# JialeTao/MRFA

Measured on AMD Instinct MI355X. Metric: frames/sec (256x256 source+driving pair) fwd+bwd, higher is better.
Workload: dtype f32; 1 GPU; vox1.yaml MTIA (TokenPose_B) prior + DenseMotion + RaftFlow refinement, 256x256, bs=8/GPU, fwd+bwd+clip+Adam, train-mode BN, surrogate L1 loss; global_batch=8, parallelism=dp1, prior=mtia, background_predictor=False, sync_bn=False, launch=hipGraph, optimizer=FlatAdam (K20), mfma=bf16x6

## Files before the change

mrfa_amd/build.py:

```python
import glob
import os
import subprocess
import sys

HERE = os.path.dirname(os.path.abspath(__file__))
ROOT = os.path.dirname(HERE)
CSRC = os.path.join(HERE, "csrc")
LIBDIR = os.path.join(HERE, "_lib")
LIB = os.path.join(LIBDIR, "libmrfa_hip.so")
SOURCES = ["error.cpp", "conv_plan.hip", "conv_mfma.hip", "conv_split.hip", "conv_halo.hip", "conv_small.hip", "conv_lean.hip", "wgrad_mfma.hip", "wgrad_split.hip", "wgrad_halo.hip", "wgrad_small.hip", "wgrad_lean.hip", "conv_fewout.hip", "conv_fewout3.hip", "layout.hip", "pack_multi.hip", "norm.hip", "sample.hip", "elementwise.hip", "optim.hip", "tokenpose.hip", "attention_mfma.hip", "losses.hip", "prior.hip", "pose.hip", "metrics.hip", "frames.hip"]
FLAGS = ["--offload-arch=gfx950", "-O3", "-std=c++17", "-fPIC", "-I" + os.path.join(ROOT, "include"), "-I" + CSRC,
         "-Wno-unused-result"]


def _stale(out, deps):
    if not os.path.exists(out):
        return True
    t = os.path.getmtime(out)
    return any(os.path.getmtime(d) > t for d in deps)


def build(force: bool = False, verbose: bool = True) -> str:
    os.makedirs(LIBDIR, exist_ok=True)
    hipcc = os.environ.get("HIPCC", "/opt/rocm/bin/hipcc")
    headers = [os.path.join(ROOT, "include", h) for h in ("mrfa_hip.h", "mrfa_hip_ext.h")] + sorted(glob.glob(os.path.join(CSRC, "*.h")))
# ... 28 lines not shown
```

mrfa_amd/csrc/common.h:

```cpp
#pragma once
#include <hip/hip_runtime.h>
#include <stdio.h>
#include <string.h>
#include "mrfa_hip.h"

typedef float f32x16 __attribute__((ext_vector_type(16)));
typedef float f32x4 __attribute__((ext_vector_type(4)));

void mrfa_set_error(const char* fmt, ...);

struct MrfaTuning {
    int conv_small_env;
    int conv_small;
    int conv_halo, conv_halo_min_tiles, conv_halo_pr, conv_halo_phase, conv_halo_bn256, conv_halo_bn192, conv_halo_bn64_fill;
    int conv_lean, conv_lean_min_wgs, conv_lean_geo, gemm_lean;
    int wgrad_halo, wgrad_halo_min_wgs, wgrad_halo_target_wgs, wgrad_halo_phase, wgrad_lean;
    int conv_fewout3, attention_mfma, split_target_256;
};
extern MrfaTuning g_tune;

struct HaloGeo { int PR, BN; bool phase; };

enum class ConvFamily { lean, gemm_lean, small, halo, halo_dgrad, rows_split, rows_f32, refused };
struct ConvPlan {
    ConvFamily family;
    char error[256];
    long long M;
    int KT;
    int lean_geo, gemm_cfg, small_tm, small_tn;
    HaloGeo halo;
    int BM, BN, splitk;
    bool w8;
    bool fused;
    bool fin_in_launch;
    bool reads_w;
    int last_config;
    bool groups_ok, bst_ok, stride2_ok, mask_ok, phase_dgrad_ok;
};
ConvPlan plan_conv(const mrfa_conv_params& p);

enum class WgradFamily { lean, small, halo, tiled, refused };
struct WgradPlan {
    WgradFamily family;
    char error[192];
    long long M;
    bool lean, small;
    bool groups_ok, stride2_ok;
};
WgradPlan plan_wgrad(const mrfa_wgrad_params& p);

int mrfa_conv_split_launch(hipStream_t st, const mrfa_conv_params& p, int KT, long long M, int splitk, int BN);
bool mrfa_conv_halo_eligible(const mrfa_conv_params& p, HaloGeo* geo);
int mrfa_conv_halo_launch(hipStream_t st, const mrfa_conv_params& p, const HaloGeo& geo);
int mrfa_wgrad_split_launch(hipStream_t st, const mrfa_wgrad_params& p, dim3 grid, long long M, long long kps, int tiles_n, int nsplit, int inner,
                            int total_splits, int taps, long long partial_stride, int BM, int BN);

bool mrfa_wgrad_halo_eligible(const mrfa_wgrad_params& p);
int mrfa_wgrad_halo_launch(hipStream_t st, const mrfa_wgrad_params& p);

bool mrfa_fewout3_wgrad(hipStream_t st, const float* x, int ldx, int N, int H, int W, int Cin, const float* dy, int lddy, int Cout, int R, int pad,
                        float* dw, float* dbias, int* rc);

int mrfa_conv_lean_pick(const mrfa_conv_params& p);
int mrfa_conv_lean_launch(hipStream_t st, const mrfa_conv_params& p, int geo);
int mrfa_gemm_lean_pick(const mrfa_conv_params& p, long long M);
int mrfa_gemm_lean_launch(hipStream_t st, const mrfa_conv_params& p, long long M, int cfg);

bool mrfa_conv_small_eligible(const mrfa_conv_params& p, long long M);
int mrfa_conv_small_launch(hipStream_t st, const mrfa_conv_params& p, long long M, int tm, int tn);

bool mrfa_attention_mfma_ok(int d, int n, const void* qkv, int ld, const void* out, int ldo, const void* dout, int lddo, const void* dqkv, int lddq);
int mrfa_attention_fwd_mfma(hipStream_t st, const float* qkv, int ld, int B, int n, int heads, int d, float scale, float* out, int ldo, float* lse);
int mrfa_attention_bwd_mfma(hipStream_t st, const float* qkv, int ld, const float* out, int ldo, const float* dout, int lddo, const float* lse,
                            float* delta, int B, int n, int heads, int d, float scale, float* dqkv, int lddq);

bool mrfa_wgrad_lean_eligible(const mrfa_wgrad_params& p);
int mrfa_wgrad_lean_multi(hipStream_t st, const mrfa_wgrad_params* ps, int n, unsigned char* taken);

bool mrfa_wgrad_small_eligible(const mrfa_wgrad_params& p, long long M);
int mrfa_wgrad_small_launch(hipStream_t st, const mrfa_wgrad_params& p, long long M);

#define MRFA_CHECK_ARG(cond, ...)                      \
    do {                                               \
        if (!(cond)) {                                 \
// ... 123 lines not shown
```

mrfa_amd/csrc/conv_mfma.hip:

```cpp
#include "common.h"
#include <stdlib.h>

namespace {

constexpr int BK = 32;
constexpr int LDK = BK + 4;

template <int BM, int BN, int WAVES_M, int WAVES_N, bool FLAT>
__global__ __launch_bounds__(WAVES_M * WAVES_N * 64) void conv_mfma_kernel(const mrfa_conv_params p, const int KT, const int kt_per_split,
                                                       const long long M, const int tiles_n, const int total_tiles) {
    constexpr int TM = BM / WAVES_M / 32;
    constexpr int TN = BN / WAVES_N / 32;
    constexpr int NT = WAVES_M * WAVES_N * 64;
    constexpr int RSTEP = NT / 8;
    constexpr int RA = BM / RSTEP;
    constexpr int RB = BN / RSTEP;
    static_assert(WAVES_M * WAVES_N == 4 || WAVES_M * WAVES_N == 8, "4 or 8 waves");
    static_assert(RA >= 1 && RB >= 1, "tile too small for the workgroup");
    static_assert(TM >= 1 && TN >= 1, "tile");

    __shared__ __attribute__((aligned(16))) float smem[2 * (BM + BN) * LDK];

    const int tid = threadIdx.x;
    const int lane = tid & 63;
// ... 375 lines not shown
    }
    if (p.bst_x) {
        MRFA_CHECK_ARG(p.stats && p.bst_scale && p.bst_shift && p.bst_mean && p.bst_invstd && !p.fin_scale,
                       "conv2d: bst_x needs stats, bst_scale / _shift / _mean / _invstd and no fin_*");
        MRFA_CHECK_ARG(c.bst_ok, "conv2d: bst_* is only implemented by the small-problem kernels: ask mrfa_conv2d_bwdstats_supported() first");
    }
    MRFA_CHECK_ARG(p.y, "conv2d: null pointer");
    if (c.family == ConvFamily::refused) { mrfa_set_error("%s", c.error); return 1; }
    int rc;
    switch (c.family) {
        case ConvFamily::lean: g_last_tile = c.last_config; rc = mrfa_conv_lean_launch(st, p, c.lean_geo); break;
        case ConvFamily::gemm_lean: g_last_tile = c.last_config; rc = mrfa_gemm_lean_launch(st, p, c.M, c.gemm_cfg); break;
        case ConvFamily::small: g_last_tile = c.last_config; rc = mrfa_conv_small_launch(st, p, c.M, c.small_tm, c.small_tn); break;
        case ConvFamily::halo:
        case ConvFamily::halo_dgrad: g_last_tile = c.last_config; rc = mrfa_conv_halo_launch(st, p, c.halo); break;
        default: rc = launch_rows(st, p, c); break;
    }
    if (rc || !p.fin_scale || c.fin_in_launch) return rc;
    return mrfa_bn_finalize_groups(stream, p.stats, p.fin_count, p.fin_gamma, p.fin_beta, p.fin_rmean, p.fin_rvar, p.fin_momentum, p.fin_eps,
                                   p.Cout, p.groups > 1 ? p.groups : 1, p.fin_scale, p.fin_shift, p.fin_mean, p.fin_invstd);
}
```

mrfa_amd/csrc/conv_plan.hip:

```cpp
#include "common.h"
#include <stdarg.h>
#include <stdlib.h>

namespace {
int env_int(const char* name, int dflt) { const char* e = getenv(name); return e ? atoi(e) : dflt; }
int env_on(const char* name) { const char* e = getenv(name); return !(e && e[0] == '0'); }
}

MrfaTuning g_tune = {
     env_on("MRFA_CONV_SMALL"),  1,
     env_on("MRFA_CONV_HALO"),  128,  0,  1,  1,
     1,  1,
     env_on("MRFA_CONV_LEAN"),  128,  -1,
     env_int("MRFA_GEMM_LEAN", 1),
     env_on("MRFA_WGRAD_HALO"),  192,  256,  1,
     env_on("MRFA_WGRAD_LEAN"),
     1,  env_on("MRFA_ATTENTION_MFMA"),  env_int("MRFA_SPLIT_TARGET_256", 1),
};

enum TuneKind { T_ON, T_INT, T_NONNEG, T_NONNEG_ON, T_LEVEL, T_POS };
static const struct { const char* key; int* field; TuneKind kind; } TUNING_KEYS[] = {
    {"conv_small", &g_tune.conv_small, T_ON},
    {"conv_halo", &g_tune.conv_halo, T_ON},
    {"conv_halo_min_tiles", &g_tune.conv_halo_min_tiles, T_INT},
    {"conv_halo_pr", &g_tune.conv_halo_pr, T_INT},
    {"conv_halo_phase", &g_tune.conv_halo_phase, T_ON},
    {"conv_halo_bn256", &g_tune.conv_halo_bn256, T_ON},
    {"conv_halo_bn192", &g_tune.conv_halo_bn192, T_ON},
    {"conv_halo_bn64_fill", &g_tune.conv_halo_bn64_fill, T_ON},
    {"conv_lean", &g_tune.conv_lean, T_ON},
    {"conv_lean_min_wgs", &g_tune.conv_lean_min_wgs, T_NONNEG},
    {"conv_lean_geo", &g_tune.conv_lean_geo, T_INT},
    {"gemm_lean", &g_tune.gemm_lean, T_LEVEL},
    {"wgrad_halo", &g_tune.wgrad_halo, T_ON},
    {"wgrad_halo_min_wgs", &g_tune.wgrad_halo_min_wgs, T_NONNEG},
    {"wgrad_halo_target_wgs", &g_tune.wgrad_halo_target_wgs, T_POS},
    {"wgrad_halo_phase", &g_tune.wgrad_halo_phase, T_NONNEG_ON},
    {"wgrad_lean", &g_tune.wgrad_lean, T_ON},
    {"conv_fewout3", &g_tune.conv_fewout3, T_ON},
    {"attention_mfma", &g_tune.attention_mfma, T_ON},
};

extern "C" int mrfa_set_tuning(const char* key, int value) {
    if (!key) return -1;
    for (const auto& k : TUNING_KEYS) {
        if (strcmp(key, k.key)) continue;
        const int prev = *k.field;
        switch (k.kind) {
            case T_ON: *k.field = value != 0; break;
            case T_INT: *k.field = value; break;
            case T_NONNEG: if (value >= 0) *k.field = value; break;
            case T_NONNEG_ON: if (value >= 0) *k.field = value != 0; break;
            case T_LEVEL: if (value >= 0) *k.field = value > 2 ? 2 : value; break;
            case T_POS: if (value > 0) *k.field = value; break;
        }
// ... 84 lines not shown
ConvPlan plan_conv(const mrfa_conv_params& p) {
    ConvPlan c = {};
    const int mode = mrfa_get_mfma_mode();
    const bool flat = p.kflat > 0;
    c.M = (long long)p.N * p.Hout * p.Wout;
    c.KT = ((flat ? p.kflat : p.R * p.S * p.Cin) + BK - 1) / BK;
    c.splitk = 1;
    c.reads_w = true;
    c.fin_in_launch = p.fin_scale != nullptr;

    c.lean_geo = flat ? -1 : mrfa_conv_lean_pick(p);
    c.gemm_cfg = (flat || c.lean_geo >= 0) ? -1 : mrfa_gemm_lean_pick(p, c.M);
    const bool lean = c.lean_geo >= 0, gemm = c.gemm_cfg >= 0;
    const bool small = !lean && !gemm && g_tune.conv_small_env && g_tune.conv_small && mrfa_conv_small_eligible(p, c.M);
    const bool halo = !flat && mrfa_conv_halo_eligible(p, &c.halo);

    const long long rows = group_rows(p, c.M);
    c.groups_ok = p.groups <= 1 || !(p.stats || p.fin_scale || p.bst_x || p.in_scale) ||
                  (p.nbatch <= 1 && p.splitk <= 1 && rows > 0 &&
                   (lean || gemm || (!p.in_scale && ((rows % 128) == 0 || small || (p.stride <= 1 && halo)))));
    c.bst_ok = p.stats && !p.fin_scale && p.stride >= 0 && !flat && (lean || gemm || small);
    c.stride2_ok = p.stride == 2 && p.Hout == (p.Hin + 2 * p.pad - p.R) / 2 + 1 && p.Wout == (p.Win + 2 * p.pad - p.S) / 2 + 1 &&
                   (flat ? (!p.ups && p.nbatch <= 1 && p.splitk <= 1 && p.ktab) : small);
    c.mask_ok = halo;
    c.phase_dgrad_ok = p.ups == 2 && halo;

    if (!(p.x && p.w)) return refuse(c, "conv2d: null pointer");
    if (!(p.N > 0 && p.Cin > 0 && p.Cout > 0 && p.Hout > 0 && p.Wout > 0)) return refuse(c, "conv2d: bad sizes");
    if (!(p.R >= 1 && p.S >= 1 && p.R <= 15 && p.S <= 15)) return refuse(c, "conv2d: kernel size %dx%d unsupported", p.R, p.S);
    if (!((p.w_ld % 4) == 0 && aligned16(p.w))) return refuse(c, "conv2d: packed weight must be 16-B aligned, w_ld %% 4 == 0");
// ... 26 lines not shown
        c.small_tn = tn;
        c.last_config = (16 << 16) | (16 << 4) | 8;
        return c;
    }
    if (p.stride < 0 || p.stride > 2 || (p.stride == 2 && !(flat && !p.ups && p.nbatch <= 1)))
        return refuse(c, "conv2d: stride = %d is only implemented by the one-wave-per-tile kernel and by flat-K launches: ask mrfa_conv2d_stride_supported() first", p.stride);
    if (p.mask && !halo) return refuse(c, "conv2d: `mask` is only honoured by the patch-tiled kernel: ask mrfa_conv2d_mask_supported() first");
    if (p.ups == 2 && !halo)
        return refuse(c, "conv2d: ups = 2 (phase data gradient of a fused-upsample layer) is only implemented for the shapes mrfa_conv2d_phase_dgrad_supported() reports");
    if (halo) {
        c.family = p.ups == 2 ? ConvFamily::halo_dgrad : ConvFamily::halo;
        c.reads_w = false;
        c.last_config = (128 << 16) | ((p.Cout <= 64 ? 64 : 128) << 4) | 4 | (1 << 28);
        return c;
    }
    plan_rows(c, p, mode);
    return c;
}

WgradPlan plan_wgrad(const mrfa_wgrad_params& p) {
    WgradPlan c = {};
    const bool flat = p.kflat > 0;
    c.M = (long long)p.N * p.Hout * p.Wout;
    c.lean = mrfa_wgrad_lean_eligible(p);
    c.small = g_tune.conv_small_env && g_tune.conv_small && mrfa_wgrad_small_eligible(p, c.M);
    c.groups_ok = p.groups <= 1 || !p.in_scale || c.lean;
    c.stride2_ok = p.stride == 2 && p.Hout == (p.Hin + 2 * p.pad - p.R) / 2 + 1 && p.Wout == (p.Win + 2 * p.pad - p.S) / 2 + 1 && c.small;
    if (!(p.x && p.dy && p.dw)) return refuse(c, "wgrad: null pointer");
    if (!flat && !((p.ldx % 4) == 0 && aligned16(p.x))) return refuse(c, "wgrad: x must be a 16-B aligned view with ld %% 4 == 0");
    if (flat && !p.ktab) return refuse(c, "wgrad: flat mode needs ktab");
    if (!(c.M < (1ll << 31) - 64)) return refuse(c, "wgrad: too many pixels");
    if (p.in_scale && c.lean) { c.family = WgradFamily::lean; return c; }
    if (!c.groups_ok) return refuse(c, "wgrad: groups = %d with a prologue is only implemented where mrfa_conv2d_wgrad_groups_supported() says so", p.groups);
    if (c.small) { c.family = WgradFamily::small; return c; }
    if (p.stride > 1) return refuse(c, "wgrad: stride = %d is only implemented by the small-problem kernel: ask mrfa_conv2d_wgrad_stride_supported() first", p.stride);
    c.family = !flat && mrfa_wgrad_halo_eligible(p) ? WgradFamily::halo : WgradFamily::tiled;
    return c;
}

extern "C" int mrfa_conv2d_split_k(const mrfa_conv_params* p) {
    if (!p) return 1;
    if (p->splitk > 1) return p->splitk;
    const ConvPlan c = plan_conv(*p);
// ... 19 lines not shown
```

mrfa_amd/csrc/pack_multi.hip:

```cpp
#include <type_traits>
#include "mfma_bf16.h"

namespace {

constexpr int TCI = 32;
constexpr int MAXD = MRFA_PACK_MAX_DESCS;
constexpr int LDS_FLOATS = 12832;

struct PackArgs {
    int n;
    int tile_prefix[MAXD + 1];
    mrfa_pack_desc d[MAXD];
};

__host__ __device__ inline int tco_for(int T) { return T <= 9 ? 32 : (T <= 25 ? 16 : 8); }
__host__ __device__ inline int rup(int a, int b) { return (a + b - 1) / b * b; }

__device__ __forceinline__ long long dst_index(int mode, int co, int ci, int t, int Cout, int Cin, int T) {
    switch (mode) {
        case 0: return ((long long)t * rup(Cout, 128) + co) * rup(Cin, 32) + ci;
        case 1: return (long long)co * rup(T * Cin, 32) + t * Cin + ci;
        case 2: return ((long long)(T - 1 - t) * rup(Cin, 128) + ci) * rup(Cout, 32) + co;
        case 3: return (long long)ci * rup(T * Cout, 32) + (T - 1 - t) * Cout + co;
        case 5: return ((long long)co * T + t) * Cin + ci;
        default: return ((long long)ci * T + (T - 1 - t)) * Cout + co;
    }
}

__device__ __forceinline__ long long chunk_major(int tt, int r, int f, int rowsP, int colsP) {
    return (long long)tt * rowsP * colsP + (long long)(f >> 4) * (rowsP * 16) + r * 16 + (f & 15);
}

__device__ __forceinline__ int find_desc(const int* prefix, int n, int b) {
    int lo = 0, hi = n - 1;
    while (lo < hi) {
        const int mid = (lo + hi + 1) >> 1;
        if (prefix[mid] <= b) lo = mid; else hi = mid - 1;
    }
    return lo;
}

__global__ __launch_bounds__(256) void pack_multi_kernel(const PackArgs a) {
    __shared__ float lds[LDS_FLOATS];
    const int di = find_desc(a.tile_prefix, a.n, blockIdx.x);
    const mrfa_pack_desc& d = a.d[di];
    const int T = d.R * d.S, Cout = d.Cout, Cin = d.Cin;
    const int TCO = tco_for(T);
    const int tiles_ci = (Cin + TCI - 1) / TCI;
    const int tile = blockIdx.x - a.tile_prefix[di];
    const int co0 = (tile / tiles_ci) * TCO, ci0 = (tile % tiles_ci) * TCI;
    const int nco = min(TCO, Cout - co0), nci = min(TCI, Cin - ci0);
    const int row = TCI * T + 1;
    const int seg = nci * T;
    for (int i = threadIdx.x; i < nco * seg; i += 256) {
        const int co_l = i / seg, r = i - co_l * seg;
        lds[co_l * row + r] = d.src[((size_t)(co0 + co_l) * Cin + ci0) * T + r];
    }
    __syncthreads();
    for (int k = 0; k < d.ndst; ++k) {
        const int mode = d.mode[k];
        float* __restrict__ dst = d.dst[k];
        if (mode == 12 || mode == 13) {
            constexpr unsigned RM[4] = {0x1u, 0x6u, 0x3u, 0x4u};
            const bool tr = mode == 13;
            unsigned short* __restrict__ d16 = reinterpret_cast<unsigned short*>(dst);
            const int rowsP = tr ? rup(Cin, 128) : rup(Cout, 128), colsP = tr ? rup(Cout, 32) : rup(Cin, 32);
            const long long piece = 16ll * rowsP * colsP;
            const int nfast = tr ? nco : nci, nslow = tr ? nci : nco;
            const int f0 = (threadIdx.x & 15) * 2;
            for (int q = threadIdx.x >> 4; q < nslow * 16; q += 16) {
                const int sl = q >> 4, pt = q & 15;
                if (f0 >= nfast) continue;
                const int ph = pt >> 2, a_ = (pt >> 1) & 1, b_ = pt & 1;
                const unsigned rm = RM[(ph >> 1) * 2 + a_], sm = RM[(ph & 1) * 2 + b_];
                float v[2] = {0.f, 0.f};
#pragma unroll
                for (int e = 0; e < 2; ++e) {
                    if (f0 + e < nfast) {
                        const int co_l = tr ? f0 + e : sl, ci_l = tr ? sl : f0 + e;
                        const float* wl = lds + co_l * row + ci_l * T;
#pragma unroll
                        for (int r = 0; r < 3; ++r)
#pragma unroll
                            for (int s_ = 0; s_ < 3; ++s_)
                                if (((rm >> r) & 1u) && ((sm >> s_) & 1u)) v[e] += wl[r * 3 + s_];
                    }
                }
                const long long idx = tr ? chunk_major(pt, ci0 + sl, co0 + f0, rowsP, colsP) : chunk_major(pt, co0 + sl, ci0 + f0, rowsP, colsP);
                float x0 = v[0], x1 = v[1];
#pragma unroll
                for (int pc = 0; pc < 3; ++pc) {
                    const unsigned b0 = __float_as_uint(x0) & 0xffff0000u, b1 = __float_as_uint(x1) & 0xffff0000u;
                    *reinterpret_cast<unsigned*>(d16 + pc * piece + idx) = (b0 >> 16) | b1;
                    x0 -= __uint_as_float(b0);
                    x1 -= __uint_as_float(b1);
                }
            }
            continue;
        }
        const bool ci_fast = mode == 0 || mode == 1 || mode == 5 || mode == 8 || mode == 14;
        const bool bf = mode == 8 || mode == 9 || mode == 14 || mode == 15;
        const bool rne1 = mode == 14 || mode == 15;
        const int nf = ci_fast ? nci : nco;
        const int lanes_f = bf ? 16 : 32;
        const int f0 = (threadIdx.x & (lanes_f - 1)) * (bf ? 2 : 1);
        const int rows_per_pass = 256 / lanes_f;
        const int r0 = threadIdx.x / lanes_f;
        const int n_inner = ci_fast ? T : nci;
        const int n_rows = ci_fast ? nco * T : T * nci;
        int outer = r0 / n_inner, inner = r0 - outer * n_inner;
        const int base_mode = (mode == 8 || mode == 14) ? 0 : ((mode == 9 || mode == 15) ? 2 : mode);
        unsigned short* __restrict__ d16 = reinterpret_cast<unsigned short*>(dst);
        const long long piece = base_mode == 0 ? (long long)T * rup(Cout, 128) * rup(Cin, 32) : (long long)T * rup(Cin, 128) * rup(Cout, 32);
        for (int q = r0; q < n_rows; q += rows_per_pass) {
            if (f0 < nf) {
                const int co_l = ci_fast ? outer : f0, t = ci_fast ? inner : outer, ci_l = ci_fast ? f0 : inner;
                const int lstep = ci_fast ? T : row;
                const float v0 = lds[co_l * row + ci_l * T + t];
                const long long idx = !bf ? dst_index(base_mode, co0 + co_l, ci0 + ci_l, t, Cout, Cin, T)
                                      : (base_mode == 0 ? chunk_major(t, co0 + co_l, ci0 + ci_l, rup(Cout, 128), rup(Cin, 32))
                                                        : chunk_major(T - 1 - t, ci0 + ci_l, co0 + co_l, rup(Cin, 128), rup(Cout, 32)));
                if (!bf) {
                    dst[idx] = v0;
                } else {
                    const bool two = f0 + 1 < nf;
                    const float v1 = two ? lds[co_l * row + ci_l * T + t + lstep] : 0.f;
                    if (rne1) {
                        const unsigned ra = rne16(v0), rb = rne16(v1);
                        if (two) *reinterpret_cast<unsigned*>(d16 + idx) = ra | (rb << 16);
                        else d16[idx] = (unsigned short)ra;
                        inner += rows_per_pass;
                        while (inner >= n_inner) { inner -= n_inner; ++outer; }
                        continue;
                    }
                    unsigned h[3], l[3];
                    float a = v0, b = v1;
#pragma unroll
                    for (int pc = 0; pc < 3; ++pc) {
                        const unsigned ba = __float_as_uint(a) & 0xffff0000u, bb = __float_as_uint(b) & 0xffff0000u;
                        l[pc] = ba >> 16;
                        h[pc] = bb >> 16;
                        a -= __uint_as_float(ba);
                        b -= __uint_as_float(bb);
                    }
#pragma unroll
                    for (int pc = 0; pc < 3; ++pc) {
                        if (two) *reinterpret_cast<unsigned*>(d16 + pc * piece + idx) = l[pc] | (h[pc] << 16);
                        else d16[pc * piece + idx] = (unsigned short)l[pc];
                    }
                }
            }
            inner += rows_per_pass;
            while (inner >= n_inner) { inner -= n_inner; ++outer; }
        }
    }
}

struct UnpackArgs {
    int n;
    int tile_prefix[MAXD + 1];
    mrfa_unpack_desc d[MAXD];
};

__global__ __launch_bounds__(256) void unpack_multi_kernel(const UnpackArgs a) {
    __shared__ float lds[LDS_FLOATS];
    const int di = find_desc(a.tile_prefix, a.n, blockIdx.x);
    const mrfa_unpack_desc& d = a.d[di];
    const int T = d.T, Cout = d.Cout, Cin = d.Cin;
    const int TCO = tco_for(T);
    const int tiles_ci = (Cin + TCI - 1) / TCI;
    const int tile = blockIdx.x - a.tile_prefix[di];
    const int co0 = (tile / tiles_ci) * TCO, ci0 = (tile % tiles_ci) * TCI;
    const int nco = min(TCO, Cout - co0), nci = min(TCI, Cin - ci0);
    const int row = TCI * T + 1;
    const int seg = nci * T;
    {
        const int ci_l = threadIdx.x & 31, r0 = threadIdx.x >> 5;
        int co_l = r0 / T, t = r0 - co_l * T;
        for (int q = r0; q < nco * T; q += 8) {
            if (ci_l < nci) {
                const size_t s = d.fewout ? ((size_t)(co0 + co_l) * T + t) * Cin + ci0 + ci_l : ((size_t)t * Cout + co0 + co_l) * Cin + ci0 + ci_l;
                lds[co_l * row + ci_l * T + t] = d.src[s];
            }
            t += 8;
            while (t >= T) { t -= T; ++co_l; }
        }
    }
    __syncthreads();
    for (int i = threadIdx.x; i < nco * seg; i += 256) {
        const int co_l = i / seg, r = i - co_l * seg;
        atomicAdd(d.dst + ((size_t)(co0 + co_l) * Cin + ci0) * T + r, lds[co_l * row + r]);
    }
}

template <typename Args, typename Desc, typename Kernel>
int launch_chunks(hipStream_t st, const Desc* descs, int n, Kernel kernel, const char* what) {
    for (int base = 0; base < n; base += MAXD) {
        Args a;
        a.n = min(MAXD, n - base);
        int tiles = 0;
// ... 41 lines not shown
```

mrfa_amd/csrc/wgrad_mfma.hip:

```cpp
#include "common.h"
#include <stdlib.h>
#include <algorithm>

namespace {

constexpr int WBK = 32;
constexpr int KG = WBK / 4;

template <int BM, int BN, int WAVES_M, int WAVES_N, bool FLAT, bool ROWAL>
__global__ __launch_bounds__(WAVES_M * WAVES_N * 64) void wgrad_mfma_kernel(const mrfa_wgrad_params p, const long long M, const long long k_per_split,
                                                        const int tiles_n, const int nsplit, const int dy_scalar,
                                                        const int inner, const int total_splits, const int taps,
                                                        const long long partial_stride) {
    constexpr int WTM = BM / WAVES_M, WTN = BN / WAVES_N;
    constexpr int TM = WTM / 32, TN = WTN / 32;
    constexpr int NT = WAVES_M * WAVES_N * 64;
    static_assert((NT == 256 || NT == 512) && TM >= 1 && TN >= 1, "tile");
    constexpr int SA = BM / 4 + 4, SB = BN / 4 + 4;
    constexpr int PLA = 4 * SA, PLB = 4 * SB;
    constexpr int IA = (BM / 4) * KG, IB = (BN / 4) * KG;
    __shared__ f32x4 smem[2 * KG * (PLA + PLB)];

    const int tid = threadIdx.x, lane = tid & 63, wave = tid >> 6;
    const int wm = wave / WAVES_N, wn = wave % WAVES_N;
// ... 303 lines not shown
        atomicAdd(dw + i, s);
    }
}

}

extern "C" int mrfa_conv2d_wgrad_nhwc(void* stream, const mrfa_wgrad_params* pp) {
    const mrfa_wgrad_params& p = *pp;
    hipStream_t st = (hipStream_t)stream;
    const WgradPlan c = plan_wgrad(p);
    const long long M = c.M;
    switch (c.family) {
        case WgradFamily::refused: mrfa_set_error("%s", c.error); return 1;
        case WgradFamily::lean: { unsigned char taken = 0; return mrfa_wgrad_lean_multi(st, &p, 1, &taken); }
        case WgradFamily::small: return mrfa_wgrad_small_launch(st, p, M);
        case WgradFamily::halo: return mrfa_wgrad_halo_launch(st, p);
        case WgradFamily::tiled: break;
    }
    const int dy_scalar = ((p.ldy % 4) == 0 && aligned16(p.dy) && (p.dy_bs % 4) == 0) ? 0 : 1;
    const bool flat = p.kflat > 0;
    const int nb = p.nbatch > 1 ? p.nbatch : 1;
    int taps = flat ? 1 : p.R * p.S;
    const int NTOT = flat ? p.kflat : p.Cin;
    auto pick = [](int n) {
        const int cands[4] = {128, 96, 64, 32};
        const double pen[4] = {1.0, 1.12, 1.35, 1.8};
        int best_t = 128;
        double best = 1e18;
        for (int i = 0; i < 4; ++i) {
            const double cost = (double)cdiv(n, cands[i]) * cands[i] * pen[i];
// ... 85 lines not shown
```

Baseline: 102.3 pairs/s.

## Add direct few-input-channel 3x3 conv and wgrad kernels, batch pack loads

Adds a new conv_fewin family: direct FP32 3x3 convolution and weight-gradient kernels for layers with 1-4 input channels. They stage an input halo strip in LDS and keep the weights or accumulators in registers, replacing the MFMA GEMM paths that are poorly utilised at such a small K. The planner routes eligible shapes to it by default. The weight pack kernels also batch 12 global loads per thread before storing to LDS, and the bf16 split-packing logic moves into a shared helper. Risks: register pressure from the per-thread accumulator arrays, atomic contention on dw, and possible regressions for mid-sized Cout.

Result: no change. 101.5 pairs/s (-0.8%).

```diff
diff --git a/mrfa_amd/build.py b/mrfa_amd/build.py
--- a/mrfa_amd/build.py
+++ b/mrfa_amd/build.py
@@ -8,7 +8,7 @@
 CSRC = os.path.join(HERE, "csrc")
 LIBDIR = os.path.join(HERE, "_lib")
 LIB = os.path.join(LIBDIR, "libmrfa_hip.so")
-SOURCES = ["error.cpp", "conv_plan.hip", "conv_mfma.hip", "conv_split.hip", "conv_halo.hip", "conv_small.hip", "conv_lean.hip", "wgrad_mfma.hip", "wgrad_split.hip", "wgrad_halo.hip", "wgrad_small.hip", "wgrad_lean.hip", "conv_fewout.hip", "conv_fewout3.hip", "layout.hip", "pack_multi.hip", "norm.hip", "sample.hip", "elementwise.hip", "optim.hip", "tokenpose.hip", "attention_mfma.hip", "losses.hip", "prior.hip", "pose.hip", "metrics.hip", "frames.hip"]
+SOURCES = ["error.cpp", "conv_plan.hip", "conv_mfma.hip", "conv_split.hip", "conv_halo.hip", "conv_small.hip", "conv_lean.hip", "wgrad_mfma.hip", "wgrad_split.hip", "wgrad_halo.hip", "wgrad_small.hip", "wgrad_lean.hip", "conv_fewout.hip", "conv_fewout3.hip", "conv_fewin.hip", "layout.hip", "pack_multi.hip", "norm.hip", "sample.hip", "elementwise.hip", "optim.hip", "tokenpose.hip", "attention_mfma.hip", "losses.hip", "prior.hip", "pose.hip", "metrics.hip", "frames.hip"]
 FLAGS = ["--offload-arch=gfx950", "-O3", "-std=c++17", "-fPIC", "-I" + os.path.join(ROOT, "include"), "-I" + CSRC,
          "-Wno-unused-result"]
 
diff --git a/mrfa_amd/csrc/common.h b/mrfa_amd/csrc/common.h
--- a/mrfa_amd/csrc/common.h
+++ b/mrfa_amd/csrc/common.h
@@ -16,12 +16,13 @@
     int conv_lean, conv_lean_min_wgs, conv_lean_geo, gemm_lean;
     int wgrad_halo, wgrad_halo_min_wgs, wgrad_halo_target_wgs, wgrad_halo_phase, wgrad_lean;
     int conv_fewout3, attention_mfma, split_target_256;
+    int conv_fewin;
 };
 extern MrfaTuning g_tune;
 
 struct HaloGeo { int PR, BN; bool phase; };
 
-enum class ConvFamily { lean, gemm_lean, small, halo, halo_dgrad, rows_split, rows_f32, refused };
+enum class ConvFamily { lean, gemm_lean, small, halo, halo_dgrad, fewin, rows_split, rows_f32, refused };
 struct ConvPlan {
     ConvFamily family;
     char error[256];
@@ -39,12 +40,12 @@
 };
 ConvPlan plan_conv(const mrfa_conv_params& p);
 
-enum class WgradFamily { lean, small, halo, tiled, refused };
+enum class WgradFamily { lean, small, fewin, halo, tiled, refused };
 struct WgradPlan {
     WgradFamily family;
     char error[192];
     long long M;
-    bool lean, small;
+    bool lean, small, fewin;
     bool groups_ok, stride2_ok;
 };
 WgradPlan plan_wgrad(const mrfa_wgrad_params& p);
@@ -68,6 +69,11 @@
 
 bool mrfa_conv_small_eligible(const mrfa_conv_params& p, long long M);
 int mrfa_conv_small_launch(hipStream_t st, const mrfa_conv_params& p, long long M, int tm, int tn);
+
+bool mrfa_conv_fewin_eligible(const mrfa_conv_params& p);
+int mrfa_conv_fewin_launch(hipStream_t st, const mrfa_conv_params& p, long long M);
+bool mrfa_wgrad_fewin_eligible(const mrfa_wgrad_params& p);
+int mrfa_wgrad_fewin_launch(hipStream_t st, const mrfa_wgrad_params& p);
 
 bool mrfa_attention_mfma_ok(int d, int n, const void* qkv, int ld, const void* out, int ldo, const void* dout, int lddo, const void* dqkv, int lddq);
 int mrfa_attention_fwd_mfma(hipStream_t st, const float* qkv, int ld, int B, int n, int heads, int d, float scale, float* out, int ldo, float* lse);
diff --git a/mrfa_amd/csrc/conv_fewin.hip b/mrfa_amd/csrc/conv_fewin.hip
--- /dev/null
+++ b/mrfa_amd/csrc/conv_fewin.hip
@@ -0,0 +1,261 @@
+#include "common.h"
+
+namespace {
+
+constexpr int TW = 64;
+constexpr int NPX = 2 * TW;
+constexpr int XROWS = 5;
+constexpr int XCOLS = (TW - 1) * 2 + 3;
+
+struct FewinGeo { int s, nq, nqp, G, PP, nsx, nsy; long long nstrips; };
+
+FewinGeo fewin_geo(int N, int Hout, int Wout, int Cout, int stride) {
+    FewinGeo g;
+    g.s = stride == 2 ? 2 : 1;
+    g.nq = (Cout + 3) / 4;
+    g.nqp = 1;
+    while (g.nqp < g.nq) g.nqp <<= 1;
+    g.G = 256 / g.nqp < NPX ? 256 / g.nqp : NPX;
+    g.PP = NPX / g.G;
+    g.nsx = (Wout + TW - 1) / TW;
+    g.nsy = (Hout + 1) / 2;
+    g.nstrips = (long long)N * g.nsy * g.nsx;
+    return g;
+}
+
+template <int CIN>
+__device__ __forceinline__ void stage_halo(f32x4* xs, const float* __restrict__ x, int ldx, int Hin, int Win, int n, int iy0, int ix0, int nrows, int ncols) {
+    for (int i = threadIdx.x; i < nrows * ncols; i += 256) {
+        const int rr = i / ncols, cc = i - rr * ncols;
+        const int iy = iy0 + rr, ix = ix0 + cc;
+        f32x4 v = {0.f, 0.f, 0.f, 0.f};
+        if (iy >= 0 && iy < Hin && ix >= 0 && ix < Win) {
+            const float* px = x + (((size_t)n * Hin + iy) * Win + ix) * (size_t)ldx;
+#pragma unroll
+            for (int ci = 0; ci < CIN; ++ci) v[ci] = px[ci];
+        }
+        xs[rr * XCOLS + cc] = v;
+    }
+}
+
+template <int CIN>
+__global__ __launch_bounds__(256) void conv_fewin_kernel(const mrfa_conv_params p, const FewinGeo g, const long long M, const int vec_y) {
+    __shared__ f32x4 xs[XROWS * XCOLS];
+    __shared__ float wl[9 * 4 * 128];
+    constexpr int K = 9 * CIN;
+    const int tid = threadIdx.x;
+    int b = blockIdx.x;
+    const int sx = b % g.nsx;
+    b /= g.nsx;
+    const int sy = b % g.nsy, n = b / g.nsy;
+    const int oy0 = sy * 2, ox0 = sx * TW;
+    const int tw = min(TW, p.Wout - ox0);
+    const int CP = g.nqp * 4;
+    for (int i = tid; i < K * CP; i += 256) {
+        const int co = i / K, k = i - co * K;
+        wl[k * CP + co] = co < p.Cout ? p.w[(size_t)co * p.w_ld + k] : 0.f;
+    }
+    stage_halo<CIN>(xs, p.x, p.ldx, p.Hin, p.Win, n, oy0 * g.s - 1, ox0 * g.s - 1, g.s + 3, (tw - 1) * g.s + 3);
+    __syncthreads();
+    const int q = tid & (g.nqp - 1), grp = tid / g.nqp;
+    const bool active = q < g.nq && grp < g.G;
+    const int c0 = q * 4;
+    f32x4 s1 = {0.f, 0.f, 0.f, 0.f}, s2 = {0.f, 0.f, 0.f, 0.f};
+    if (active) {
+        f32x4 wr[K];
+#pragma unroll
+        for (int k = 0; k < K; ++k) wr[k] = *reinterpret_cast<const f32x4*>(wl + k * CP + c0);
+        f32x4 bias = {0.f, 0.f, 0.f, 0.f};
+        if (p.bias) {
+#pragma unroll
+            for (int e = 0; e < 4; ++e) if (c0 + e < p.Cout) bias[e] = p.bias[c0 + e];
+        }
+        const int p0 = grp * g.PP;
+        const int pr = p0 / TW, oy = oy0 + pr;
+        if (oy < p.Hout) {
+            for (int j = 0; j < g.PP; ++j) {
+                const int pc = (p0 & (TW - 1)) + j;
+                if (pc >= tw) break;
+                const f32x4* xp = xs + (pr * g.s) * XCOLS + pc * g.s;
+                f32x4 acc = {0.f, 0.f, 0.f, 0.f};
+#pragma unroll
+                for (int t = 0; t < 9; ++t) {
+                    const f32x4 xv = xp[(t / 3) * XCOLS + (t % 3)];
+#pragma unroll
+                    for (int ci = 0; ci < CIN; ++ci) acc += wr[t * CIN + ci] * xv[ci];
+                }
+                acc += bias;
+                float* dst = p.y + (((size_t)n * p.Hout + oy) * p.Wout + ox0 + pc) * (size_t)p.ldy + c0;
+                if (vec_y && c0 + 3 < p.Cout) {
+                    *reinterpret_cast<f32x4*>(dst) = acc;
+                } else {
+#pragma unroll
+                    for (int e = 0; e < 4; ++e) {
+                        if (c0 + e < p.Cout) dst[e] = acc[e]; else acc[e] = 0.f;
+                    }
+                }
+                s1 += acc;
+                s2 += acc * acc;
+            }
+        }
+    }
+    if (p.stats) {
+        __syncthreads();
+        float* red = wl;
+        if (grp < g.G && q < g.nqp) {
+            *reinterpret_cast<f32x4*>(red + grp * CP + c0) = s1;
+            *reinterpret_cast<f32x4*>(red + (g.G + grp) * CP + c0) = s2;
+        }
+        __syncthreads();
+        if (tid < p.Cout) {
+            float t1 = 0.f, t2 = 0.f;
+            for (int r = 0; r < g.G; ++r) { t1 += red[r * CP + tid]; t2 += red[(g.G + r) * CP + tid]; }
+            const long long m0 = ((long long)n * p.Hout + oy0) * p.Wout + ox0;
+            double* st = stat_slot(p, stat_group(p, m0, M), blockIdx.x);
+            atomicAdd(st + tid, (double)t1);
+            atomicAdd(st + p.Cout + tid, (double)t2);
+        }
+    }
+}
+
+template <int CIN>
+__global__ __launch_bounds__(256) void wgrad_fewin_kernel(const mrfa_wgrad_params p, const FewinGeo g, const int vec_dy) {
+    __shared__ f32x4 xs[XROWS * XCOLS];
+    __shared__ float red[CIN * 256 * 4];
+    constexpr int K = 9 * CIN;
+    const int tid = threadIdx.x;
+    const int q = tid & (g.nqp - 1), grp = tid / g.nqp;
+    const bool active = q < g.nq && grp < g.G;
+    const int c0 = q * 4;
+    const int CP = g.nqp * 4;
+    const int p0 = grp * g.PP;
+    const int pr = p0 / TW, pc0 = p0 & (TW - 1);
+    f32x4 acc[K];
+#pragma unroll
+    for (int k = 0; k < K; ++k) acc[k] = f32x4{0.f, 0.f, 0.f, 0.f};
+    f32x4 bacc = {0.f, 0.f, 0.f, 0.f};
+    for (long long st = blockIdx.x; st < g.nstrips; st += gridDim.x) {
+        long long b = st;
+        const int sx = (int)(b % g.nsx);
+        b /= g.nsx;
+        const int sy = (int)(b % g.nsy), n = (int)(b / g.nsy);
+        const int oy0 = sy * 2, ox0 = sx * TW;
+        const int tw = min(TW, p.Wout - ox0);
+        __syncthreads();
+        stage_halo<CIN>(xs, p.x, p.ldx, p.Hin, p.Win, n, oy0 * g.s - 1, ox0 * g.s - 1, g.s + 3, (tw - 1) * g.s + 3);
+        __syncthreads();
+        const int oy = oy0 + pr;
+        if (!active || oy >= p.Hout) continue;
+        const float* dyrow = p.dy + (((size_t)n * p.Hout + oy) * p.Wout + ox0) * (size_t)p.ldy + c0;
+        for (int j0 = 0; j0 < g.PP; j0 += 4) {
+            f32x4 dv[4];
+#pragma unroll
+            for (int u = 0; u < 4; ++u) {
+                const int pc = pc0 + j0 + u;
+                dv[u] = f32x4{0.f, 0.f, 0.f, 0.f};
+                if (j0 + u < g.PP && pc < tw) {
+                    const float* src = dyrow + (size_t)pc * p.ldy;
+                    if (vec_dy && c0 + 3 < p.Cout) {
+                        dv[u] = *reinterpret_cast<const f32x4*>(src);
+                    } else {
+#pragma unroll
+                        for (int e = 0; e < 4; ++e) if (c0 + e < p.Cout) dv[u][e] = src[e];
+                    }
+                }
+            }
+#pragma unroll
+            for (int u = 0; u < 4; ++u) {
+                const int pc = pc0 + j0 + u;
+                if (j0 + u < g.PP && pc < tw) {
+                    const f32x4* xp = xs + (pr * g.s) * XCOLS + pc * g.s;
+#pragma unroll
+                    for (int t = 0; t < 9; ++t) {
+                        const f32x4 xv = xp[(t / 3) * XCOLS + (t % 3)];
+#pragma unroll
+                        for (int ci = 0; ci < CIN; ++ci) acc[t * CIN + ci] += dv[u] * xv[ci];
+                    }
+                    bacc += dv[u];
+                }
+            }
+        }
+    }
+    const bool writer = grp < g.G;
+#pragma unroll
+    for (int t = 0; t < 9; ++t) {
+        __syncthreads();
+        if (writer) {
+#pragma unroll
+            for (int ci = 0; ci < CIN; ++ci) *reinterpret_cast<f32x4*>(red + (ci * g.G + grp) * CP + c0) = acc[t * CIN + ci];
+        }
+        __syncthreads();
+        for (int o = tid; o < CIN * CP; o += 256) {
+            const int ci = o / CP, co = o - ci * CP;
+            if (co >= p.Cout) continue;
+            float sum = 0.f;
+            for (int r = 0; r < g.G; ++r) sum += red[(ci * g.G + r) * CP + co];
+            atomicAdd(p.dw + ((size_t)t * p.Cout + co) * p.Cin + ci, sum * p.alpha);
+        }
+    }
+    if (p.dbias) {
+        __syncthreads();
+        if (writer) *reinterpret_cast<f32x4*>(red + grp * CP + c0) = bacc;
+        __syncthreads();
+        if (tid < p.Cout) {
+            float sum = 0.f;
+            for (int r = 0; r < g.G; ++r) sum += red[r * CP + tid];
+            atomicAdd(p.dbias + tid, sum);
+        }
+    }
+}
+
+bool fewin_shape(int Cin, int Cout, int R, int S, int pad, int stride, int ups, int Hin, int Win, int Hout, int Wout) {
+    if (Cin < 1 || Cin > 4 || Cout < 1 || Cout > 128 || R != 3 || S != 3 || pad != 1 || ups) return false;
+    if (stride == 2) return Hout == (Hin - 1) / 2 + 1 && Wout == (Win - 1) / 2 + 1;
+    return (stride == 0 || stride == 1) && Hout == Hin && Wout == Win;
+}
+
+}
+
+bool mrfa_conv_fewin_eligible(const mrfa_conv_params& p) {
+    if (!g_tune.conv_fewin || !fewin_shape(p.Cin, p.Cout, p.R, p.S, p.pad, p.stride, p.ups, p.Hin, p.Win, p.Hout, p.Wout)) return false;
+    if (p.kflat != 9 * p.Cin || p.w_ld < p.kflat || p.ldx < p.Cin || p.ldy < p.Cout) return false;
+    if (p.in_scale || p.out_scale || p.res || p.relu || p.mask || p.accumulate || p.alpha != 1.f || p.bst_x) return false;
+    if (p.nbatch > 1 || p.splitk > 1 || p.tile || p.w_phase) return false;
+    if (p.groups > 1 && p.stats && (p.N % p.groups) != 0) return false;
+    return true;
+}
+
+int mrfa_conv_fewin_launch(hipStream_t st, const mrfa_conv_params& p, long long M) {
+    const FewinGeo g = fewin_geo(p.N, p.Hout, p.Wout, p.Cout, p.stride);
+    const int vec_y = (p.ldy % 4) == 0 && aligned16(p.y);
+    const dim3 grid((unsigned)g.nstrips);
+    switch (p.Cin) {
+        case 1: hipLaunchKernelGGL(conv_fewin_kernel<1>, grid, dim3(256), 0, st, p, g, M, vec_y); break;
+        case 2: hipLaunchKernelGGL(conv_fewin_kernel<2>, grid, dim3(256), 0, st, p, g, M, vec_y); break;
+        case 3: hipLaunchKernelGGL(conv_fewin_kernel<3>, grid, dim3(256), 0, st, p, g, M, vec_y); break;
+        default: hipLaunchKernelGGL(conv_fewin_kernel<4>, grid, dim3(256), 0, st, p, g, M, vec_y); break;
+    }
+    MRFA_CHECK_LAUNCH("mrfa_conv2d_nhwc(fewin)");
+    return 0;
+}
+
+bool mrfa_wgrad_fewin_eligible(const mrfa_wgrad_params& p) {
+    if (!g_tune.conv_fewin || !fewin_shape(p.Cin, p.Cout, p.R, p.S, p.pad, p.stride, p.ups, p.Hin, p.Win, p.Hout, p.Wout)) return false;
+    if (p.kflat != 0 && p.kflat != 9 * p.Cin) return false;
+    if (p.in_scale || p.nbatch > 1 || p.ldx < p.Cin || p.ldy < p.Cout) return false;
+    return true;
+}
+
+int mrfa_wgrad_fewin_launch(hipStream_t st, const mrfa_wgrad_params& p) {
+    const FewinGeo g = fewin_geo(p.N, p.Hout, p.Wout, p.Cout, p.stride);
+    const int vec_dy = (p.ldy % 4) == 0 && aligned16(p.dy);
+    const dim3 grid((unsigned)(g.nstrips < 512 ? g.nstrips : 512));
+    switch (p.Cin) {
+        case 1: hipLaunchKernelGGL(wgrad_fewin_kernel<1>, grid, dim3(256), 0, st, p, g, vec_dy); break;
+        case 2: hipLaunchKernelGGL(wgrad_fewin_kernel<2>, grid, dim3(256), 0, st, p, g, vec_dy); break;
+        case 3: hipLaunchKernelGGL(wgrad_fewin_kernel<3>, grid, dim3(256), 0, st, p, g, vec_dy); break;
+        default: hipLaunchKernelGGL(wgrad_fewin_kernel<4>, grid, dim3(256), 0, st, p, g, vec_dy); break;
+    }
+    MRFA_CHECK_LAUNCH("mrfa_conv2d_wgrad_nhwc(fewin)");
+    return 0;
+}
diff --git a/mrfa_amd/csrc/conv_mfma.hip b/mrfa_amd/csrc/conv_mfma.hip
--- a/mrfa_amd/csrc/conv_mfma.hip
+++ b/mrfa_amd/csrc/conv_mfma.hip
@@ -413,6 +413,7 @@
         case ConvFamily::small: g_last_tile = c.last_config; rc = mrfa_conv_small_launch(st, p, c.M, c.small_tm, c.small_tn); break;
         case ConvFamily::halo:
         case ConvFamily::halo_dgrad: g_last_tile = c.last_config; rc = mrfa_conv_halo_launch(st, p, c.halo); break;
+        case ConvFamily::fewin: g_last_tile = c.last_config; rc = mrfa_conv_fewin_launch(st, p, c.M); break;
         default: rc = launch_rows(st, p, c); break;
     }
     if (rc || !p.fin_scale || c.fin_in_launch) return rc;
diff --git a/mrfa_amd/csrc/conv_plan.hip b/mrfa_amd/csrc/conv_plan.hip
--- a/mrfa_amd/csrc/conv_plan.hip
+++ b/mrfa_amd/csrc/conv_plan.hip
@@ -16,6 +16,7 @@
      env_on("MRFA_WGRAD_HALO"),  192,  256,  1,
      env_on("MRFA_WGRAD_LEAN"),
      1,  env_on("MRFA_ATTENTION_MFMA"),  env_int("MRFA_SPLIT_TARGET_256", 1),
+     1,
 };
 
 enum TuneKind { T_ON, T_INT, T_NONNEG, T_NONNEG_ON, T_LEVEL, T_POS };
@@ -39,6 +40,7 @@
     {"wgrad_lean", &g_tune.wgrad_lean, T_ON},
     {"conv_fewout3", &g_tune.conv_fewout3, T_ON},
     {"attention_mfma", &g_tune.attention_mfma, T_ON},
+    {"conv_fewin", &g_tune.conv_fewin, T_ON},
 };
 
 extern "C" int mrfa_set_tuning(const char* key, int value) {
@@ -153,6 +155,7 @@
     const bool lean = c.lean_geo >= 0, gemm = c.gemm_cfg >= 0;
     const bool small = !lean && !gemm && g_tune.conv_small_env && g_tune.conv_small && mrfa_conv_small_eligible(p, c.M);
     const bool halo = !flat && mrfa_conv_halo_eligible(p, &c.halo);
+    const bool fewin = flat && mrfa_conv_fewin_eligible(p);
 
     const long long rows = group_rows(p, c.M);
     c.groups_ok = p.groups <= 1 || !(p.stats || p.fin_scale || p.bst_x || p.in_scale) ||
@@ -209,6 +212,12 @@
         c.last_config = (128 << 16) | ((p.Cout <= 64 ? 64 : 128) << 4) | 4 | (1 << 28);
         return c;
     }
+    if (fewin) {
+        c.family = ConvFamily::fewin;
+        c.fin_in_launch = false;
+        c.last_config = (2 << 16) | (64 << 4) | 2 | (1 << 25);
+        return c;
+    }
     plan_rows(c, p, mode);
     return c;
 }
@@ -219,9 +228,11 @@
     c.M = (long long)p.N * p.Hout * p.Wout;
     c.lean = mrfa_wgrad_lean_eligible(p);
     c.small = g_tune.conv_small_env && g_tune.conv_small && mrfa_wgrad_small_eligible(p, c.M);
+    c.fewin = !c.small && mrfa_wgrad_fewin_eligible(p);
     c.groups_ok = p.groups <= 1 || !p.in_scale || c.lean;
-    c.stride2_ok = p.stride == 2 && p.Hout == (p.Hin + 2 * p.pad - p.R) / 2 + 1 && p.Wout == (p.Win + 2 * p.pad - p.S) / 2 + 1 && c.small;
+    c.stride2_ok = p.stride == 2 && p.Hout == (p.Hin + 2 * p.pad - p.R) / 2 + 1 && p.Wout == (p.Win + 2 * p.pad - p.S) / 2 + 1 && (c.small || c.fewin);
     if (!(p.x && p.dy && p.dw)) return refuse(c, "wgrad: null pointer");
+    if (c.fewin && c.M < (1ll << 31) - 64) { c.family = WgradFamily::fewin; return c; }
     if (!flat && !((p.ldx % 4) == 0 && aligned16(p.x))) return refuse(c, "wgrad: x must be a 16-B aligned view with ld %% 4 == 0");
     if (flat && !p.ktab) return refuse(c, "wgrad: flat mode needs ktab");
     if (!(c.M < (1ll << 31) - 64)) return refuse(c, "wgrad: too many pixels");
diff --git a/mrfa_amd/csrc/pack_lines.h b/mrfa_amd/csrc/pack_lines.h
--- /dev/null
+++ b/mrfa_amd/csrc/pack_lines.h
@@ -0,0 +1,106 @@
+#pragma once
+#include <stdint.h>
+
+#if defined(__HIPCC__)
+#define PL_HD __host__ __device__ __forceinline__
+#else
+#define PL_HD inline
+#endif
+
+struct alignas(16) PlU4 { unsigned x, y, z, w; };
+
+struct PlTile {
+    int T, Cout, Cin;
+    int co0, ci0, nco, nci;
+    int row;
+};
+
+PL_HD int pl_tco_for(int T) { return T <= 9 ? 32 : (T <= 25 ? 16 : 8); }
+PL_HD int pl_rup(int a, int b) { return (a + b - 1) / b * b; }
+PL_HD unsigned pl_bits(float x) { return __builtin_bit_cast(unsigned, x); }
+PL_HD float pl_float(unsigned u) { return __builtin_bit_cast(float, u); }
+PL_HD unsigned pl_rne16(float x) {
+    const unsigned u = pl_bits(x);
+    return (u + 0x7fffu + ((u >> 16) & 1u)) >> 16;
+}
+PL_HD long long pl_chunk_major(int tt, int r, int f, int rowsP, int colsP) {
+    return (long long)tt * rowsP * colsP + (long long)(f >> 4) * (rowsP * 16) + r * 16 + (f & 15);
+}
+
+PL_HD float pl_phase_weight(const float* wl, int pt) {
+    const unsigned RM = 0x4361u;
+    const int ph = pt >> 2, a_ = (pt >> 1) & 1, b_ = pt & 1;
+    const unsigned rm = (RM >> (4 * ((ph >> 1) * 2 + a_))) & 0xfu, sm = (RM >> (4 * ((ph & 1) * 2 + b_))) & 0xfu;
+    float v = 0.f;
+    for (int r = 0; r < 3; ++r)
+        for (int s_ = 0; s_ < 3; ++s_)
+            if (((rm >> r) & 1u) && ((sm >> s_) & 1u)) v += wl[r * 3 + s_];
+    return v;
+}
+
+PL_HD void pack_lines_store(const float* lds, const PlTile& tl, int mode, unsigned short* d16, int tid, int nthreads) {
+    const bool phase = mode == 12 || mode == 13;
+    const bool tr = mode == 9 || mode == 15 || mode == 13;
+    const int np = (mode == 14 || mode == 15) ? 1 : 3;
+    const int T = tl.T, NT = phase ? 16 : T;
+    const int rowsP = tr ? pl_rup(tl.Cin, 128) : pl_rup(tl.Cout, 128), colsP = tr ? pl_rup(tl.Cout, 32) : pl_rup(tl.Cin, 32);
+    const long long piece = (long long)NT * rowsP * colsP;
+    const int nfast = tr ? tl.nco : tl.nci, nslow = tr ? tl.nci : tl.nco;
+    const int r0 = tr ? tl.ci0 : tl.co0, f0 = tr ? tl.co0 : tl.ci0;
+    const int ftile = tr ? pl_tco_for(T) : 32;
+    const int OC = ftile >= 16 ? 2 : 1, NC = ftile >= 16 ? ftile / 16 : 1;
+    const int nitems = NT * NC * nslow * OC;
+    const bool al16 = (reinterpret_cast<uintptr_t>(d16) & 15u) == 0;
+    for (int i = tid; i < nitems; i += nthreads) {
+        const int h = i % OC;
+        int j = i / OC;
+        const int sl = j % nslow;
+        j /= nslow;
+        const int c = j % NC, tp = j / NC;
+        const int fl = c * 16 + h * 8;
+        if (fl >= nfast) continue;
+        const int nv = nfast - fl < 8 ? nfast - fl : 8;
+        unsigned short pc[3][8];
+#pragma unroll
+        for (int e = 0; e < 8; ++e) {
+            float v = 0.f;
+            if (e < nv) {
+                const int co_l = tr ? fl + e : sl, ci_l = tr ? sl : fl + e;
+                const float* wl = lds + co_l * tl.row + ci_l * T;
+                v = phase ? pl_phase_weight(wl, tp) : wl[tp];
+            }
+            if (np == 1) {
+                pc[0][e] = (unsigned short)pl_rne16(v);
+            } else {
+#pragma unroll
+                for (int k = 0; k < 3; ++k) {
+                    const unsigned b = pl_bits(v) & 0xffff0000u;
+                    pc[k][e] = (unsigned short)(b >> 16);
+                    v -= pl_float(b);
+                }
+            }
+        }
+        const int tt = phase ? tp : (tr ? T - 1 - tp : tp);
+        const long long idx = pl_chunk_major(tt, r0 + sl, f0 + fl, rowsP, colsP);
+#pragma unroll
+        for (int k = 0; k < 3; ++k) {
+            if (k >= np) break;
+            unsigned short* dst = d16 + k * piece + idx;
+            if (nv == 8 && al16) {
+                PlU4 u;
+                u.x = pc[k][0] | ((unsigned)pc[k][1] << 16);
+                u.y = pc[k][2] | ((unsigned)pc[k][3] << 16);
+                u.z = pc[k][4] | ((unsigned)pc[k][5] << 16);
+                u.w = pc[k][6] | ((unsigned)pc[k][7] << 16);
+                *reinterpret_cast<PlU4*>(dst) = u;
+            } else {
+#pragma unroll
+                for (int e = 0; e < 8; e += 2) {
+                    if (e >= nv) break;
+                    if (e + 1 < nv || phase) *reinterpret_cast<unsigned*>(dst + e) = pc[k][e] | ((unsigned)pc[k][e + 1] << 16);
+                    else dst[e] = pc[k][e];
+                }
+            }
+        }
+    }
+}
diff --git a/mrfa_amd/csrc/pack_multi.hip b/mrfa_amd/csrc/pack_multi.hip
--- a/mrfa_amd/csrc/pack_multi.hip
+++ b/mrfa_amd/csrc/pack_multi.hip
@@ -1,5 +1,6 @@
 #include <type_traits>
 #include "mfma_bf16.h"
+#include "pack_lines.h"
 
 namespace {
 
@@ -27,9 +28,6 @@
     }
 }
 
-__device__ __forceinline__ long long chunk_major(int tt, int r, int f, int rowsP, int colsP) {
-    return (long long)tt * rowsP * colsP + (long long)(f >> 4) * (rowsP * 16) + r * 16 + (f & 15);
-}
 
 __device__ __forceinline__ int find_desc(const int* prefix, int n, int b) {
     int lo = 0, hi = n - 1;
@@ -52,105 +50,44 @@
     const int nco = min(TCO, Cout - co0), nci = min(TCI, Cin - ci0);
     const int row = TCI * T + 1;
     const int seg = nci * T;
-    for (int i = threadIdx.x; i < nco * seg; i += 256) {
-        const int co_l = i / seg, r = i - co_l * seg;
-        lds[co_l * row + r] = d.src[((size_t)(co0 + co_l) * Cin + ci0) * T + r];
+    constexpr int LOAD_BATCH = 12;
+    for (int i0 = threadIdx.x; i0 < nco * seg; i0 += 256 * LOAD_BATCH) {
+        float v[LOAD_BATCH];
+#pragma unroll
+        for (int u = 0; u < LOAD_BATCH; ++u) {
+            const int i = i0 + u * 256;
+            const int co_l = i / seg, r = i - co_l * seg;
+            v[u] = i < nco * seg ? d.src[((size_t)(co0 + co_l) * Cin + ci0) * T + r] : 0.f;
+        }
+#pragma unroll
+        for (int u = 0; u < LOAD_BATCH; ++u) {
+            const int i = i0 + u * 256;
+            const int co_l = i / seg, r = i - co_l * seg;
+            if (i < nco * seg) lds[co_l * row + r] = v[u];
+        }
     }
     __syncthreads();
     for (int k = 0; k < d.ndst; ++k) {
         const int mode = d.mode[k];
         float* __restrict__ dst = d.dst[k];
-        if (mode == 12 || mode == 13) {
-            constexpr unsigned RM[4] = {0x1u, 0x6u, 0x3u, 0x4u};
-            const bool tr = mode == 13;
-            unsigned short* __restrict__ d16 = reinterpret_cast<unsigned short*>(dst);
-            const int rowsP = tr ? rup(Cin, 128) : rup(Cout, 128), colsP = tr ? rup(Cout, 32) : rup(Cin, 32);
-            const long long piece = 16ll * rowsP * colsP;
-            const int nfast = tr ? nco : nci, nslow = tr ? nci : nco;
-            const int f0 = (threadIdx.x & 15) * 2;
-            for (int q = threadIdx.x >> 4; q < nslow * 16; q += 16) {
-                const int sl = q >> 4, pt = q & 15;
-                if (f0 >= nfast) continue;
-                const int ph = pt >> 2, a_ = (pt >> 1) & 1, b_ = pt & 1;
-                const unsigned rm = RM[(ph >> 1) * 2 + a_], sm = RM[(ph & 1) * 2 + b_];
-                float v[2] = {0.f, 0.f};
-#pragma unroll
-                for (int e = 0; e < 2; ++e) {
-                    if (f0 + e < nfast) {
-                        const int co_l = tr ? f0 + e : sl, ci_l = tr ? sl : f0 + e;
-                        const float* wl = lds + co_l * row + ci_l * T;
-#pragma unroll
-                        for (int r = 0; r < 3; ++r)
-#pragma unroll
-                            for (int s_ = 0; s_ < 3; ++s_)
-                                if (((rm >> r) & 1u) && ((sm >> s_) & 1u)) v[e] += wl[r * 3 + s_];
-                    }
-                }
-                const long long idx = tr ? chunk_major(pt, ci0 + sl, co0 + f0, rowsP, colsP) : chunk_major(pt, co0 + sl, ci0 + f0, rowsP, colsP);
-                float x0 = v[0], x1 = v[1];
-#pragma unroll
-                for (int pc = 0; pc < 3; ++pc) {
-                    const unsigned b0 = __float_as_uint(x0) & 0xffff0000u, b1 = __float_as_uint(x1) & 0xffff0000u;
-                    *reinterpret_cast<unsigned*>(d16 + pc * piece + idx) = (b0 >> 16) | b1;
-                    x0 -= __uint_as_float(b0);
-                    x1 -= __uint_as_float(b1);
-                }
-            }
+        if (mode >= 8) {
+            const PlTile tl = {T, Cout, Cin, co0, ci0, nco, nci, row};
+            pack_lines_store(lds, tl, mode, reinterpret_cast<unsigned short*>(dst), (int)threadIdx.x, 256);
             continue;
         }
-        const bool ci_fast = mode == 0 || mode == 1 || mode == 5 || mode == 8 || mode == 14;
-        const bool bf = mode == 8 || mode == 9 || mode == 14 || mode == 15;
-        const bool rne1 = mode == 14 || mode == 15;
+        const bool ci_fast = mode == 0 || mode == 1 || mode == 5;
         const int nf = ci_fast ? nci : nco;
-        const int lanes_f = bf ? 16 : 32;
-        const int f0 = (threadIdx.x & (lanes_f - 1)) * (bf ? 2 : 1);
-        const int rows_per_pass = 256 / lanes_f;
-        const int r0 = threadIdx.x / lanes_f;
+        const int f0 = threadIdx.x & 31;
+        const int r0 = threadIdx.x >> 5;
         const int n_inner = ci_fast ? T : nci;
         const int n_rows = ci_fast ? nco * T : T * nci;
         int outer = r0 / n_inner, inner = r0 - outer * n_inner;
-        const int base_mode = (mode == 8 || mode == 14) ? 0 : ((mode == 9 || mode == 15) ? 2 : mode);
-        unsigned short* __restrict__ d16 = reinterpret_cast<unsigned short*>(dst);
-        const long long piece = base_mode == 0 ? (long long)T * rup(Cout, 128) * rup(Cin, 32) : (long long)T * rup(Cin, 128) * rup(Cout, 32);
-        for (int q = r0; q < n_rows; q += rows_per_pass) {
+        for (int q = r0; q < n_rows; q += 8) {
             if (f0 < nf) {
                 const int co_l = ci_fast ? outer : f0, t = ci_fast ? inner : outer, ci_l = ci_fast ? f0 : inner;
-                const int lstep = ci_fast ? T : row;
-                const float v0 = lds[co_l * row + ci_l * T + t];
-                const long long idx = !bf ? dst_index(base_mode, co0 + co_l, ci0 + ci_l, t, Cout, Cin, T)
-                                      : (base_mode == 0 ? chunk_major(t, co0 + co_l, ci0 + ci_l, rup(Cout, 128), rup(Cin, 32))
-                                                        : chunk_major(T - 1 - t, ci0 + ci_l, co0 + co_l, rup(Cin, 128), rup(Cout, 32)));
-                if (!bf) {
-                    dst[idx] = v0;
-                } else {
-                    const bool two = f0 + 1 < nf;
-                    const float v1 = two ? lds[co_l * row + ci_l * T + t + lstep] : 0.f;
-                    if (rne1) {
-                        const unsigned ra = rne16(v0), rb = rne16(v1);
-                        if (two) *reinterpret_cast<unsigned*>(d16 + idx) = ra | (rb << 16);
-                        else d16[idx] = (unsigned short)ra;
-                        inner += rows_per_pass;
-                        while (inner >= n_inner) { inner -= n_inner; ++outer; }
-                        continue;
-                    }
-                    unsigned h[3], l[3];
-                    float a = v0, b = v1;
-#pragma unroll
-                    for (int pc = 0; pc < 3; ++pc) {
-                        const unsigned ba = __float_as_uint(a) & 0xffff0000u, bb = __float_as_uint(b) & 0xffff0000u;
-                        l[pc] = ba >> 16;
-                        h[pc] = bb >> 16;
-                        a -= __uint_as_float(ba);
-                        b -= __uint_as_float(bb);
-                    }
-#pragma unroll
-                    for (int pc = 0; pc < 3; ++pc) {
-                        if (two) *reinterpret_cast<unsigned*>(d16 + pc * piece + idx) = l[pc] | (h[pc] << 16);
-                        else d16[pc * piece + idx] = (unsigned short)l[pc];
-                    }
-                }
+                dst[dst_index(mode, co0 + co_l, ci0 + ci_l, t, Cout, Cin, T)] = lds[co_l * row + ci_l * T + t];
             }
-            inner += rows_per_pass;
+            inner += 8;
             while (inner >= n_inner) { inner -= n_inner; ++outer; }
         }
     }
@@ -175,15 +112,23 @@
     const int row = TCI * T + 1;
     const int seg = nci * T;
     {
+        constexpr int LOAD_BATCH = 12;
         const int ci_l = threadIdx.x & 31, r0 = threadIdx.x >> 5;
-        int co_l = r0 / T, t = r0 - co_l * T;
-        for (int q = r0; q < nco * T; q += 8) {
-            if (ci_l < nci) {
+        for (int q0 = r0; q0 < nco * T; q0 += 8 * LOAD_BATCH) {
+            float v[LOAD_BATCH];
+#pragma unroll
+            for (int u = 0; u < LOAD_BATCH; ++u) {
+                const int q = q0 + 8 * u;
+                const int co_l = q / T, t = q - co_l * T;
                 const size_t s = d.fewout ? ((size_t)(co0 + co_l) * T + t) * Cin + ci0 + ci_l : ((size_t)t * Cout + co0 + co_l) * Cin + ci0 + ci_l;
-                lds[co_l * row + ci_l * T + t] = d.src[s];
+                v[u] = (q < nco * T && ci_l < nci) ? d.src[s] : 0.f;
             }
-            t += 8;
-            while (t >= T) { t -= T; ++co_l; }
+#pragma unroll
+            for (int u = 0; u < LOAD_BATCH; ++u) {
+                const int q = q0 + 8 * u;
+                const int co_l = q / T, t = q - co_l * T;
+                if (q < nco * T && ci_l < nci) lds[co_l * row + ci_l * T + t] = v[u];
+            }
         }
     }
     __syncthreads();
diff --git a/mrfa_amd/csrc/wgrad_mfma.hip b/mrfa_amd/csrc/wgrad_mfma.hip
--- a/mrfa_amd/csrc/wgrad_mfma.hip
+++ b/mrfa_amd/csrc/wgrad_mfma.hip
@@ -341,6 +341,7 @@
         case WgradFamily::refused: mrfa_set_error("%s", c.error); return 1;
         case WgradFamily::lean: { unsigned char taken = 0; return mrfa_wgrad_lean_multi(st, &p, 1, &taken); }
         case WgradFamily::small: return mrfa_wgrad_small_launch(st, p, M);
+        case WgradFamily::fewin: return mrfa_wgrad_fewin_launch(st, p);
         case WgradFamily::halo: return mrfa_wgrad_halo_launch(st, p);
         case WgradFamily::tiled: break;
     }
```
